# yang-z-03/scd-resnet

Hardware: AMD Instinct MI355X
Metric: 512x512 images/sec training, centerOffsetRes10, at 1/2/4/8 MI355X (higher is better)
Workload: dtype bf16; 1 GPU; centerOffsetRes10 train step (fwd+focal/L1 loss+bwd+Adam, DDP over RCCL), 512x512 synthetic SCD tiles; model=centerOffsetRes10, global_batch=32, step_issue=eager launches, per_gpu_batch=32, parallelism=dp1, image_size=512

## Files before the change

include/scdhip.h:

```cpp
#ifndef SCDHIP_H
#define SCDHIP_H
#include <stddef.h>
#include <stdint.h>

#ifdef __cplusplus
extern "C" {
#endif

#define SCD_DT_F32 0
#define SCD_DT_BF16 1
#define SCD_DT_F16 2

#define SCD_ERR_ARG 9001

#define SCD_MAX_TAPS 16
#define SCD_MAX_PHASES 4
#define SCD_STAT_REPLICAS 64

typedef struct scd_gemm_phase {
    int Qh, Qw, rho_h, rho_w, ntaps;
    int dh[SCD_MAX_TAPS], dw[SCD_MAX_TAPS], wt[SCD_MAX_TAPS];
} scd_gemm_phase;

int scd_conv_gemm(int dtype, const void* x, const void* w, void* y, const float* bias, double* stats,
                  int N, int Hi, int Wi, int Ci, int Ho, int Wo, int Co, int in_stride, int out_stride,
                  int wrow, int relu, int accumulate, int nphase, const scd_gemm_phase* phases,
                  void* stream);

int scd_conv_dgrad_s2(int dtype, const void* dy, const void* w3, void* dx, int N, int Hq, int Wq, int Cg, int Cin,
                      int accumulate, void* stream);
int scd_conv_gemm_bnbwd(int dtype, const void* x, const void* w, void* y, int N, int Hi, int Wi, int Ci, int Ho,
                        int Wo, int Co, int in_stride, int out_stride, int wrow, int nphase,
                        const scd_gemm_phase* phases, const void* bn_y, const float* mean, const float* invstd,
                        const float* relu_scale, const float* relu_shift, double* bn_stats, void* stream);
int scd_conv_gemm_res(int dtype, const void* x, const void* w, void* y, const float* bias, const void* res, int N,
                      int Hi, int Wi, int Ci, int Ho, int Wo, int Co, int in_stride, int out_stride, int wrow,
                      int relu, int nphase, const scd_gemm_phase* phases, void* stream);
int scd_conv_gemm_heads(int dtype, const void* x, const void* w, void* hid, const float* bias, int N, int H,
                        int W, int Ci, int nh, const int* od, const float* const* w1, const float* const* b1,
                        float* const* outs, void* stream);
int scd_conv_gemm_heads_keep(int dtype, const void* x, const void* w, void* hid, const float* bias, int N, int H,
                             int W, int Ci, int nh, const int* od, const float* const* w1, const float* const* b1,
                             float* const* outs, const unsigned char* keep, int keep_cols, void* stream);

size_t scd_conv_wgrad_workspace(int Cg, int T, int Ci, int nsplit);
int scd_conv_wgrad_nsplit(int dtype, long M, int Cg, int T, int Ci);
int scd_conv_wgrad_nsplit2(int dtype, long M, int Ho, int Wo, int Cg, int T, int Ci);
int scd_conv_wgrad(int dtype, const void* g, const void* x, float* ws, int nsplit,
                   int N, int Ho, int Wo, int Cg, int Hi, int Wi, int Ci, int in_stride,
                   int T, const int* dh, const int* dw, void* stream);
int scd_wgrad_reduce(const float* ws, int nsplit, int Cg, int T, int Ci, int r0, int r1, int cvalid,
                     long ld_n, long ld_c, long ld_t, float* dst, int accumulate, float alpha, void* stream);
int scd_wgrad_reduce_rows(const float* ws, int nsplit, int Cg, int T, int Ci, int nslices, const int* r0,
                          const int* r1, const long* ld_n, const long* ld_c, const long* ld_t, float* const* dst,
                          int cvalid, int accumulate, float alpha, void* stream);

int scd_pack_weight(int dtype, const float* w, void* out, int A, int B, int T, int mode, int ldp,
                    int row_off, void* stream);

int scd_pad_channels(int dtype, const void* src, long rows, int C, int Cp, void* dst, void* stream);

int scd_upsample2x_add(int dtype, const void* up, const void* low, void* out, int N, int h, int w, int C, void* stream);
int scd_upsample2x_add_bwd(int dtype, const void* dout, void* dlow, int N, int h, int w, int C, void* stream);

typedef struct scd_pack_desc {
    const float* w;
    void* out;
    long start;
    int A, B, T, mode, ldp, row_off, a_off, a_tot;
} scd_pack_desc;
int scd_pack_weights_batched(int dtype, const scd_pack_desc* descs, int n, long total, void* stream);

int scd_im2col_stem(int dtype, const float* x, void* cols, int N, int H, int W, int Ho, int Wo, int kh,
                    int kw, int stride, int pad, int Kpad, void* stream);

int scd_stem_conv_fwd(int dtype, const float* x, const void* wpk, void* y, double* stats, int N, int H, int W,
                      int Ho, int Wo, void* stream);
int scd_stem_conv_wgrad_nsplit(long M);
int scd_stem_conv_wgrad(int dtype, const void* dy, const void* ybn, const float* coef, const float* x, float* ws,
                        int nsplit, int N, int H, int W, int Ho, int Wo, void* stream);
int scd_stem_bwd_nsplit(void);
int scd_stem_bwd_fused(int dtype, const void* dout, const uint8_t* argmax, const void* y, const float* scale,
                       const float* shift, const float* mean, const float* invstd, const float* x, double* stats,
                       float* ws, int nsplit, float* tg, int N, int H, int W, int Ho, int Wo, void* stream);
int scd_stem_bwd_combine(int dtype, const float* tg, const void* wpk, const float* coef, float* dst, int accumulate,
                         float alpha, void* stream);

int scd_stats_collapse(double* stats, int nrep, int C, void* stream);
int scd_stats_collapse_to(double* stats, int nrep, int C, double* out, void* stream);
int scd_bn_finalize(double* stats, int nrep, int C, double count, const float* gamma,
                    const float* beta, float* running_mean, float* running_var, int64_t* num_batches,
                    float momentum, float eps, float* mean, float* invstd, float* scale, float* shift,
                    void* stream);
#define SCD_BN_FIN_MAX 4
typedef struct scd_bn_fin_args {
    double* stats;
    int nrep, C;
    double count;
    const float* gamma;
    const float* beta;
    float* running_mean;
    float* running_var;
    int64_t* num_batches;
    float momentum, eps;
    float* mean;
    float* invstd;
    float* scale;
    float* shift;
} scd_bn_fin_args;
int scd_bn_finalize_n(const scd_bn_fin_args* layers, int n, void* stream);
int scd_bn_apply(int dtype, const void* y, void* out, int C, long total, const float* scale,
                 const float* shift, const void* res, const float* rscale, const float* rshift,
                 int relu, void* stream);
int scd_bn_bwd_reduce(int dtype, const void* dout, const void* mask, const void* y, const float* relu_scale,
                      const float* relu_shift, const float* mean, const float* invstd, int C, long total,
                      double* stats, void* stream);
int scd_bn_bwd_finalize(double* stats, int nrep, int C, double count, const float* gamma,
// ... 189 lines not shown
```

scd-resnet_amd/csrc/conv_gemm.hip:

```cpp
#include <stdlib.h>

#include <algorithm>
#include <type_traits>

#include "gemm_common.h"
#include "scd_common.h"

#ifndef SCD_ABLATE
#define SCD_ABLATE 0
#endif

extern unsigned long long* scd_calib_stamp_buffer;

namespace {
SCD_KERNEL_NS_BEGIN

struct GemmParams {
    const char* x;
    const char* w;
    char* y;
    const float* bias;
    double* stats;
    int N, Hi, Wi, Ci, Ho, Wo, Co;
    int is, os, wrow, relu, accumulate, nphase, ntn;
// ... 819 lines not shown
        b_row[j] = b_ok[j] ? nn : 0;
    }
    const int cpt = p.Ci / BK;
    const int KT = ph.ntaps * cpt;
    const __amdgpu_buffer_rsrc_t xrs = buf_rsrc(p.x, p.xbytes);
    const __amdgpu_buffer_rsrc_t wrs = buf_rsrc(p.w, p.wbytes);

    struct StageArgs { int live, c0, dh, dw, wt; };
    auto stage_args = [&](int kt_req) {
        StageArgs a;
        a.live = kt_req < KT;
        const int kt = min(kt_req, KT - 1);
        const int chunk = kt / ph.ntaps, tap = kt - chunk * ph.ntaps;
        a.c0 = chunk * BK + cch * EPC;
        a.dh = ph.dh[tap]; a.dw = ph.dw[tap]; a.wt = ph.wt[tap];
        return a;
    };
    auto issue = [&](const StageArgs& g, int slot) {
        char* As = smem + slot * STAGE;
        char* Bs = As + BM * 128;
#pragma unroll
        for (int i = 0; i < 4; ++i) {
            const int ih = a_ih[i] + g.dh, iw = a_iw[i] + g.dw;
            const bool ok = g.live && a_ok[i] && (unsigned)ih < (unsigned)p.Hi && (unsigned)iw < (unsigned)p.Wi;
            dma16(xrs, As + (32 * wave + 8 * i) * 128, sel_off(ok, ((a_pix[i] + ih * p.Wi + iw) * p.Ci + g.c0) * 2));
        }
#pragma unroll
        for (int j = 0; j < 2; ++j)
            dma16(wrs, Bs + (16 * wave + 8 * j) * 128,
                  sel_off(g.live && b_ok[j], (b_row[j] * p.wrow + g.wt * p.Ci + g.c0) * 2));
    };

    const int wm = wave / WN, wn = wave - (wave / WN) * WN;
    const int l16 = lane & 15, lg = lane >> 4;
    const int l7 = l16 & 7;
    f32x4 acc[4][4];
#pragma unroll
    for (int a = 0; a < 4; ++a)
#pragma unroll
        for (int b = 0; b < 4; ++b) acc[a][b] = (f32x4){0.f, 0.f, 0.f, 0.f};

    issue(stage_args(0), 0);
    issue(stage_args(1), 1);
    int slot = 0;
    for (int kt = 0; kt < KT; ++kt) {
        const StageArgs nxt = stage_args(kt + 2);
        asm volatile("s_waitcnt vmcnt(6)" ::: "memory");
        __builtin_amdgcn_s_barrier();
        asm volatile("" ::: "memory");
        if constexpr (SCD_ABLATE == 2) asm volatile("s_waitcnt vmcnt(0)" ::: "memory");
        else issue(nxt, slot == 0 ? 2 : slot - 1);
        const char* As = smem + slot * STAGE;
        const char* Bs = As + BM * 128;
        h16x8 af[2][4], bfr[2][4];
#pragma unroll
        for (int s = 0; s < 2; ++s) {
            const int co = ((s * 4 + lg) ^ l7) << 4;
#pragma unroll
            for (int a = 0; a < 4; ++a) af[s][a] = *(const h16x8*)(As + (wm * 64 + a * 16 + l16) * 128 + co);
#pragma unroll
            for (int b = 0; b < 4; ++b) bfr[s][b] = *(const h16x8*)(Bs + (wn * 64 + b * 16 + l16) * 128 + co);
        }
        if constexpr (SCD_ABLATE == 1) {
#pragma unroll
            for (int s = 0; s < 2; ++s)
#pragma unroll
                for (int a = 0; a < 4; ++a) acc[a][0][0] += (float)af[s][a][0] + (float)bfr[s][a][0];
        } else {
            __builtin_amdgcn_s_setprio(1);
#pragma unroll
            for (int s = 0; s < 2; ++s)
#pragma unroll
                for (int a = 0; a < 4; ++a)
#pragma unroll
                    for (int b = 0; b < 4; ++b)
                        acc[a][b] = mfma_16x16x32_h16(bfr[s][b], af[s][a], acc[a][b]);
            __builtin_amdgcn_s_setprio(0);
        }
        slot = slot == 2 ? 0 : slot + 1;
    }
    asm volatile("s_waitcnt vmcnt(0)" ::: "memory");
    __syncthreads();
    gemm_epilogue<T, BM, BN, WN, HEADS, BNB, RES>(p, acc, smem, tid, bid, mt, nt, M, QQ, ph);
}

template <int BN, bool HEADS, bool BNB = false, bool RES = false>
__global__ __launch_bounds__(512, 1) void conv_gemm_pp_kernel(GemmParams p) {
    typedef h16 T;
    constexpr int BM = 256, BK = 64, EPC = 8;
    constexpr int NB = BN / 64;
    constexpr int WCOLS = BN / 4;
    constexpr int NB2 = (BN / 2 - 64) / 32;
    constexpr int STAGE = (BM + BN) * 128;
    constexpr int EROW = WCOLS * 2 + 16;
    constexpr int EPI = 8 * 128 * EROW;
    constexpr int EPX = EPI + 4 * BN * 4 + (HEADS ? 256 * 8 * 4 : 0);
    constexpr int SMEM = (2 * STAGE > EPX) ? 2 * STAGE : EPX;
    static_assert(BN == 256 || BN == 192, "BN");
    __shared__ __attribute__((aligned(16))) char smem[SMEM];

    const int tid = threadIdx.x;
    const int lane = tid & 63;
    const int wave = __builtin_amdgcn_readfirstlane(tid >> 6);
    const int grp = wave >> 2, wc = wave & 3;
    const int bid = xcd_tile_id();
    const GemmTile tile = gemm_tile(p, bid);
    const scd_gemm_phase& ph = p.ph[tile.phase];
    const int mt = tile.mt, nt = tile.nt, QQ = tile.QQ, M = tile.M;

    const int lrow = lane >> 3;
    const int cch = (lane & 7) ^ lrow;
    int a_base[4];
    unsigned a_mask[4];
#pragma unroll
    for (int i = 0; i < 4; ++i) {
        const int m = mt * BM + 128 * grp + 64 * (i >> 1) + 16 * wc + 8 * (i & 1) + lrow;
        const bool ok = m < M;
        const PixPos q = pix_of(ok ? m : 0, QQ, ph.Qw);
        const int ih0 = p.is * q.qh, iw0 = p.is * q.qw;
        a_base[i] = ((q.n * p.Hi + ih0) * p.Wi + iw0) * p.Ci * 2 + cch * EPC * 2;
        unsigned msk = 0;
        for (int t = 0; t < ph.ntaps; ++t) {
            const int ih = ih0 + ph.dh[t], iw = iw0 + ph.dw[t];
            if (ok && (unsigned)ih < (unsigned)p.Hi && (unsigned)iw < (unsigned)p.Wi) msk |= 1u << t;
        }
        a_mask[i] = msk;
    }
    int b_base[2 + NB2];
    bool b_ok[2 + NB2];
#pragma unroll
    for (int j = 0; j < 2 + NB2; ++j) {
        const int r = (BN / 2) * grp + (j < 2 ? 16 * wc + 8 * j : 64 + 8 * NB2 * wc + 8 * (j - 2)) + lrow;
        const int nn = nt * BN + r;
        b_ok[j] = nn < p.Co;
        b_base[j] = ((b_ok[j] ? nn : 0) * p.wrow + cch * EPC) * 2;
    }
    const int cpt = p.Ci / BK;
    const int KT = ph.ntaps * cpt;
    const __amdgpu_buffer_rsrc_t xrs = buf_rsrc(p.x, p.xbytes);
    const __amdgpu_buffer_rsrc_t wrs = buf_rsrc(p.w, p.wbytes);

    struct StageArgs { int live, tap, adelta, bdelta; };
    auto stage_args = [&](int kt_req) {
        StageArgs a;
        a.live = kt_req < KT;
        const int kt = min(kt_req, KT - 1);
        const int chunk = kt / ph.ntaps, tap = kt - chunk * ph.ntaps;
        a.tap = tap;
        a.adelta = ((ph.dh[tap] * p.Wi + ph.dw[tap]) * p.Ci + chunk * BK) * 2;
        a.bdelta = (ph.wt[tap] * p.Ci + chunk * BK) * 2;
        return a;
    };
    auto issue_a = [&](const StageArgs& g, char* buf, int h) {
#pragma unroll
        for (int j = 0; j < 2; ++j) {
            const int i = 2 * h + j;
            const bool ok = g.live && ((a_mask[i] >> g.tap) & 1u);
            dma16(xrs, buf + (128 * grp + 64 * h + 16 * wc + 8 * j) * 128, sel_off(ok, a_base[i] + g.adelta));
        }
    };
    auto issue_b = [&](const StageArgs& g, char* buf, int part) {
        char* Bs = buf + BM * 128;
#pragma unroll
        for (int j = (part ? 2 : 0); j < (part ? 2 + NB2 : 2); ++j) {
            const int r = (BN / 2) * grp + (j < 2 ? 16 * wc + 8 * j : 64 + 8 * NB2 * wc + 8 * (j - 2));
            dma16(wrs, Bs + r * 128, sel_off(g.live && b_ok[j], b_base[j] + g.bdelta));
// ... 1845 lines not shown
        if (bn == 256) hipLaunchKernelGGL((conv_gemm_pp_kernel<256, false, true>), dim3(tiles), dim3(512), 0, st, p);
        else hipLaunchKernelGGL((conv_gemm_pp_kernel<192, false, true>), dim3(tiles), dim3(512), 0, st, p);
    } else if (p.res) {
        if (bn == 256) hipLaunchKernelGGL((conv_gemm_pp_kernel<256, false, false, true>), dim3(tiles), dim3(512), 0, st, p);
        else hipLaunchKernelGGL((conv_gemm_pp_kernel<192, false, false, true>), dim3(tiles), dim3(512), 0, st, p);
    } else {
        if (bn == 256) hipLaunchKernelGGL((conv_gemm_pp_kernel<256, false>), dim3(tiles), dim3(512), 0, st, p);
        else hipLaunchKernelGGL((conv_gemm_pp_kernel<192, false>), dim3(tiles), dim3(512), 0, st, p);
    }
    SCD_RETURN_LAUNCH();
}

static int halo64_taps(const GemmParams& p, int nphase, const scd_gemm_phase* phases) {
    if (nphase != 1 || p.Ci != 64 || p.Co != 64 || p.is != 1 || p.os != 1 || p.head_on || p.wrow != 9 * 64) return -1;
    const scd_gemm_phase& ph = phases[0];
    if (ph.ntaps != 9 || ph.rho_h || ph.rho_w || ph.Qh != p.Ho || ph.Qw != p.Wo || p.Hi != p.Ho || p.Wi != p.Wo)
        return -1;
    if (p.Wo != 256 && p.Wo != 128 && p.Wo != 64) return -1;
    if (p.Wo < 256 && ph.Qh % (256 / p.Wo)) return -1;
    int fwd = 1, bwd = 1;
    for (int t = 0; t < 9; ++t) {
        const int r = t / 3, c = t % 3;
        if (ph.wt[t] != t) return -1;
        fwd &= ph.dh[t] == r - 1 && ph.dw[t] == c - 1;
        bwd &= ph.dh[t] == 1 - r && ph.dw[t] == 1 - c;
    }
    return fwd ? 0 : (bwd ? 1 : -1);
}

static int launch_l1p(int dtype, GemmParams& p, int nphase, const scd_gemm_phase* phases, long ,
                      hipStream_t st) {
    const int flip = halo64_taps(p, nphase, phases);
    const bool l1res = p.resmode && (p.bias || p.relu || p.res);
    if (dtype != SCD_DT_BF16 || flip < 0 || !halo64_mode() ||
        !(l1res ? (flip == 0 && !p.stats && !p.accumulate && !p.bnbwd) : (!p.bias && !p.relu && !p.res)))
        return -1;
    if (p.Wo == 256 && p.bnbwd) return SCD_ERR_ARG;
    const int tiles = fill_tiles(p, nphase, phases, 256, 1);
    if (!fill_ranges(dtype, p, l1res)) return SCD_ERR_ARG;
    const int tpi = p.Wo >= 256 ? p.Ho : p.Ho / (256 / p.Wo);
    int run = 1;
    while (run < 16 && tpi % (2 * run) == 0 && tiles / (2 * run) >= num_cus()) run *= 2;
    const int grid = tiles / run;
#define SCD_L1P_LAUNCH(WO)                                                                                              \
    do {                                                                                                                 \
        if (l1res) {                                                                                                     \
            hipLaunchKernelGGL((conv_gemm_l1p_kernel<WO, false, false, true>), dim3(grid), dim3(512), 0, st, p, run);    \
        } else if (WO != 256 && p.bnbwd) {                                                                                      \
            if (flip) hipLaunchKernelGGL((conv_gemm_l1p_kernel<WO, true, WO != 256>), dim3(grid), dim3(512), 0, st, p, run); \
            else hipLaunchKernelGGL((conv_gemm_l1p_kernel<WO, false, WO != 256>), dim3(grid), dim3(512), 0, st, p, run);    \
        } else {                                                                                                         \
            if (flip) hipLaunchKernelGGL((conv_gemm_l1p_kernel<WO, true, false>), dim3(grid), dim3(512), 0, st, p, run);  \
            else hipLaunchKernelGGL((conv_gemm_l1p_kernel<WO, false, false>), dim3(grid), dim3(512), 0, st, p, run);     \
        }                                                                                                                \
    } while (0)
    if (p.Wo == 256) SCD_L1P_LAUNCH(256);
    else if (p.Wo == 128) SCD_L1P_LAUNCH(128);
    else SCD_L1P_LAUNCH(64);
#undef SCD_L1P_LAUNCH
    SCD_RETURN_LAUNCH();
}

static int launch_ring(int dtype, GemmParams& p, int nphase, const scd_gemm_phase* phases, long Mtot,
                       hipStream_t st) {
    if (dtype != SCD_DT_BF16) return -1;
    bool ring;
    if (p.Co > 64) {
        const int rm = ring_mode();
        ring = rm >= 0 ? rm != 0 : cdiv(Mtot, 256) * cdiv(p.Co, 128) >= 256;
    } else {
        ring = nphase == 1 && phases[0].ntaps == 1 && p.Ci >= 128 && cdiv(Mtot, 256) >= 256;
    }
    if (!ring) return -1;
    const int tiles = fill_tiles(p, nphase, phases, 256, cdiv(p.Co, 128));
    if (tiles == 0) return 0;
    if (!fill_ranges(dtype, p, false)) return SCD_ERR_ARG;
    if (p.head_on) hipLaunchKernelGGL((conv_gemm_ring_kernel<true>), dim3(tiles), dim3(512), 0, st, p);
    else if (p.bnbwd) hipLaunchKernelGGL((conv_gemm_ring_kernel<false, true>), dim3(tiles), dim3(512), 0, st, p);
    else if (p.res) hipLaunchKernelGGL((conv_gemm_ring_kernel<false, false, true>), dim3(tiles), dim3(512), 0, st, p);
    else hipLaunchKernelGGL((conv_gemm_ring_kernel<false>), dim3(tiles), dim3(512), 0, st, p);
    SCD_RETURN_LAUNCH();
}

static int launch_tiled(int dtype, GemmParams& p, int nphase, const scd_gemm_phase* phases, long ,
                        hipStream_t st) {
    const bool narrow = p.Co <= 64;
    const int tiles = fill_tiles(p, nphase, phases, narrow ? 256 : 128, cdiv(p.Co, narrow ? 64 : 128));
    if (tiles == 0) return 0;
    if (!fill_ranges(dtype, p, false)) return SCD_ERR_ARG;
    return scd_dispatch_dtype(dtype, [&](auto tag) {
        using T = typename decltype(tag)::type;
        if (narrow) return launch_gemm<T, 256, 64>(p, tiles, st);
        int ks = 1;
        if (sizeof(T) == 2 && !p.head_on) {
            int kt = 0;
            for (int i = 0; i < nphase; ++i) kt = std::max(kt, phases[i].ntaps * (p.Ci / 64));
            if (kt >= 16 && 2 * (long)tiles <= 3L * num_cus()) ks = 2;
        }
        return launch_gemm<T, 128, 128>(p, tiles, st, ks);
    });
}

static int conv_gemm_launch(int dtype, GemmParams& p, int nphase, const scd_gemm_phase* phases, void* stream) {
    if (nphase < 1 || nphase > SCD_MAX_PHASES) return SCD_ERR_ARG;
    const int BK = dtype == SCD_DT_BF16 ? 64 : 32;
    const int EPC = dtype == SCD_DT_BF16 ? 8 : 4;
    if (p.Ci % BK != 0 || p.Co <= 0 || p.Co % EPC != 0 || p.N <= 0) return SCD_ERR_ARG;
    p.nphase = nphase;
    if (p.head_on && (p.Co <= 64 || p.Co != 128 * ((p.Co + 127) / 128))) return SCD_ERR_ARG;
    long Mtot = 0;
    for (int i = 0; i < nphase; ++i) {
        if (phases[i].ntaps < 0 || phases[i].ntaps > SCD_MAX_TAPS) return SCD_ERR_ARG;
        for (int t = 0; t < phases[i].ntaps; ++t)
            if (phases[i].wt[t] < 0 || (long)(phases[i].wt[t] + 1) * p.Ci > p.wrow) return SCD_ERR_ARG;
        Mtot += (long)p.N * phases[i].Qh * phases[i].Qw;
    }
    hipStream_t st = (hipStream_t)stream;
    int rc = launch_stream1x1(dtype, p, nphase, phases, Mtot, st);
    if (rc < 0 && stream1x1_mode() == 2) return SCD_ERR_ARG;
    if (rc < 0) rc = launch_heads384(dtype, p, nphase, phases, Mtot, st);
    if (rc < 0) rc = launch_pp(dtype, p, nphase, phases, Mtot, st);
    if (rc >= 0) return rc;
    if (p.bnbwd && dtype != SCD_DT_BF16) return SCD_ERR_ARG;
    rc = launch_l1p(dtype, p, nphase, phases, Mtot, st);
    if (rc < 0) rc = launch_ring(dtype, p, nphase, phases, Mtot, st);
    if (rc < 0) rc = launch_tiled(dtype, p, nphase, phases, Mtot, st);
    return rc;
}

static void fill_params(GemmParams& p, const void* x, const void* w, void* y, const float* bias, double* stats, int N,
                        int Hi, int Wi, int Ci, int Ho, int Wo, int Co, int in_stride, int out_stride, int wrow,
                        int relu, int accumulate) {
    p.x = (const char*)x; p.w = (const char*)w; p.y = (char*)y; p.bias = bias; p.stats = stats;
    p.N = N; p.Hi = Hi; p.Wi = Wi; p.Ci = Ci; p.Ho = Ho; p.Wo = Wo; p.Co = Co;
    p.is = in_stride; p.os = out_stride; p.wrow = wrow; p.relu = relu; p.accumulate = accumulate;
    p.ybytes = 0;
    p.head_on = 0;
    p.bnbwd = 0; p.bny = nullptr; p.bn_mean = p.bn_invstd = p.bn_rsc = p.bn_rsh = nullptr;
    p.hid_keep = nullptr; p.hid_cols = 1 << 30;
    p.shuf = 0;
    p.stamps = scd_calib_stamp_buffer;
    p.res = nullptr; p.resmode = 0;
    p.kserp = heads_serp_mode();
    for (int h = 0; h < 4; ++h) { p.head_od[h] = 0; p.head_w[h] = nullptr; p.head_b[h] = nullptr; p.head_out[h] = nullptr; }
}

extern "C" int scd_conv_gemm(int dtype, const void* x, const void* w, void* y, const float* bias, double* stats,
                             int N, int Hi, int Wi, int Ci, int Ho, int Wo, int Co, int in_stride, int out_stride,
                             int wrow, int relu, int accumulate, int nphase, const scd_gemm_phase* phases,
                             void* stream) {
    SCD_F16_FWD(scd_conv_gemm, x, w, y, bias, stats, N, Hi, Wi, Ci, Ho, Wo, Co, in_stride, out_stride, wrow, relu,
                accumulate, nphase, phases, stream);
    GemmParams p;
    fill_params(p, x, w, y, bias, stats, N, Hi, Wi, Ci, Ho, Wo, Co, in_stride, out_stride, wrow, relu, accumulate);
    return conv_gemm_launch(dtype, p, nphase, phases, stream);
}

extern "C" int scd_conv_gemm_res(int dtype, const void* x, const void* w, void* y, const float* bias, const void* res,
                                 int N, int Hi, int Wi, int Ci, int Ho, int Wo, int Co, int in_stride, int out_stride,
                                 int wrow, int relu, int nphase, const scd_gemm_phase* phases, void* stream) {
    SCD_F16_FWD(scd_conv_gemm_res, x, w, y, bias, res, N, Hi, Wi, Ci, Ho, Wo, Co, in_stride, out_stride, wrow, relu,
                nphase, phases, stream);
    if (res && res == y) return SCD_ERR_ARG;
    GemmParams p;
    fill_params(p, x, w, y, bias, nullptr, N, Hi, Wi, Ci, Ho, Wo, Co, in_stride, out_stride, wrow, relu, 0);
    p.res = (const char*)res; p.resmode = 1;
    return conv_gemm_launch(dtype, p, nphase, phases, stream);
}

extern "C" int scd_conv_gemm_bnbwd(int dtype, const void* x, const void* w, void* y, int N, int Hi, int Wi, int Ci,
                                   int Ho, int Wo, int Co, int in_stride, int out_stride, int wrow, int nphase,
                                   const scd_gemm_phase* phases, const void* bn_y, const float* mean,
                                   const float* invstd, const float* relu_scale, const float* relu_shift,
                                   double* bn_stats, void* stream) {
    SCD_F16_FWD(scd_conv_gemm_bnbwd, x, w, y, N, Hi, Wi, Ci, Ho, Wo, Co, in_stride, out_stride, wrow, nphase, phases,
                bn_y, mean, invstd, relu_scale, relu_shift, bn_stats, stream);
    if (!bn_y || !mean || !invstd || !relu_scale || !relu_shift || !bn_stats || Co % 4) return SCD_ERR_ARG;
    GemmParams p;
    fill_params(p, x, w, y, nullptr, bn_stats, N, Hi, Wi, Ci, Ho, Wo, Co, in_stride, out_stride, wrow, 0, 0);
    p.bnbwd = 1;
    p.bny = (const char*)bn_y; p.bn_mean = mean; p.bn_invstd = invstd; p.bn_rsc = relu_scale; p.bn_rsh = relu_shift;
    if (dtype == SCD_DT_BF16) {
        const int rc = conv_gemm_launch(dtype, p, nphase, phases, stream);
        if (rc != SCD_ERR_ARG) return rc;
    }
    fill_params(p, x, w, y, nullptr, nullptr, N, Hi, Wi, Ci, Ho, Wo, Co, in_stride, out_stride, wrow, 0, 0);
    const int rc = conv_gemm_launch(dtype, p, nphase, phases, stream);
    if (rc) return rc;
    return scd_bn_bwd_reduce(dtype, y, nullptr, bn_y, relu_scale, relu_shift, mean, invstd, Co, (long)N * Ho * Wo * Co,
                             bn_stats, stream);
}

extern "C" int scd_conv_dgrad_s2(int dtype, const void* dy, const void* w3, void* dx, int N, int Hq, int Wq, int Cg,
                                 int Cin, int accumulate, void* stream) {
    SCD_F16_FWD(scd_conv_dgrad_s2, dy, w3, dx, N, Hq, Wq, Cg, Cin, accumulate, stream);
    const int Co = 4 * Cin;
    if (!pp_tile_bn(dtype, Co, (long)N * Hq * Wq) || Cin % 8) return SCD_ERR_ARG;
    GemmParams p;
    fill_params(p, dy, w3, dx, nullptr, nullptr, N, Hq, Wq, Cg, Hq, Wq, Co, 1, 1, 4 * Cg, 0, accumulate);
    p.shuf = 1;
    scd_gemm_phase ph;
    ph.Qh = Hq; ph.Qw = Wq; ph.rho_h = 0; ph.rho_w = 0; ph.ntaps = 4;
    for (int t = 0; t < 4; ++t) { ph.dh[t] = t >> 1; ph.dw[t] = t & 1; ph.wt[t] = t; }
    return conv_gemm_launch(dtype, p, 1, &ph, stream);
}

extern "C" int scd_conv_gemm_heads(int dtype, const void* x, const void* w, void* hid, const float* bias, int N,
                                   int H, int W, int Ci, int nh, const int* od, const float* const* w1,
                                   const float* const* b1, float* const* outs, void* stream) {
    SCD_F16_FWD(scd_conv_gemm_heads, x, w, hid, bias, N, H, W, Ci, nh, od, w1, b1, outs, stream);
    return scd_conv_gemm_heads_keep(dtype, x, w, hid, bias, N, H, W, Ci, nh, od, w1, b1, outs, nullptr, 0, stream);
}

extern "C" int scd_conv_gemm_heads_keep(int dtype, const void* x, const void* w, void* hid, const float* bias, int N,
                                        int H, int W, int Ci, int nh, const int* od, const float* const* w1,
                                        const float* const* b1, float* const* outs, const unsigned char* keep,
                                        int keep_cols, void* stream) {
    SCD_F16_FWD(scd_conv_gemm_heads_keep, x, w, hid, bias, N, H, W, Ci, nh, od, w1, b1, outs, keep, keep_cols, stream);
    if (nh < 1 || nh > 4 || (keep && (keep_cols < 0 || keep_cols % 128))) return SCD_ERR_ARG;
    GemmParams p;
    fill_params(p, x, w, hid, bias, nullptr, N, H, W, Ci, H, W, nh * 128, 1, 1, 9 * Ci, 1, 0);
    if (keep) { p.hid_keep = keep; p.hid_cols = keep_cols; }
    p.head_on = 1;
    for (int h = 0; h < nh; ++h) {
        if (od[h] < 1 || od[h] > 4) return SCD_ERR_ARG;
        p.head_od[h] = od[h]; p.head_w[h] = w1[h]; p.head_b[h] = b1[h]; p.head_out[h] = outs[h];
    }
    scd_gemm_phase ph;
    ph.Qh = H; ph.Qw = W; ph.rho_h = 0; ph.rho_w = 0; ph.ntaps = 9;
    for (int t = 0; t < 9; ++t) { ph.dh[t] = t / 3 - 1; ph.dw[t] = t % 3 - 1; ph.wt[t] = t; }
    return conv_gemm_launch(dtype, p, 1, &ph, stream);
}

static void wgrad_tile(int Cg, int& tm, int& tn) {
    if (Cg <= 64) { tm = 64; tn = 256; }
    else { tm = 128; tn = 128; }
}

// ... 284 lines not shown
```

scd-resnet_amd/csrc/scd_common.h:

```cpp
#pragma once
#include <hip/hip_runtime.h>
#include <stdint.h>
#include <string.h>

#include "../../include/scdhip.h"

#define SCD_F16_ENTRY_POINTS(X) \
    X(scd_conv_gemm) \
    X(scd_conv_gemm_bnbwd) \
    X(scd_conv_gemm_res) \
    X(scd_conv_gemm_heads) \
    X(scd_conv_gemm_heads_keep) \
    X(scd_conv_wgrad_nsplit2) \
    X(scd_conv_wgrad_nsplit) \
    X(scd_conv_wgrad) \
    X(scd_bn_apply) \
    X(scd_bn_bwd_reduce) \
    X(scd_bn_bwd_apply) \
    X(scd_bn_bwd_reduce2) \
    X(scd_bn_bwd_apply2) \
    X(scd_pack_weights_batched) \
    X(scd_pack_weight) \
    X(scd_im2col_stem) \
    X(scd_stem_pool_fwd) \
    X(scd_stem_pool_bwd) \
    X(scd_stem_pool_bwd_bn) \
    X(scd_heads_fwd) \
    X(scd_heads_bwd) \
    X(scd_heads_bwd_packed) \
    X(scd_heads_bwd_packed_split) \
    X(scd_heads_sparse_bwd) \
    X(scd_heads_sparse_fixup) \
    X(scd_stem_conv_fwd) \
    X(scd_stem_conv_wgrad) \
    X(scd_stem_bwd_fused) \
    X(scd_conv_dgrad_s2) \
    X(scd_stem_bwd_combine) \
    X(scd_pad_channels) \
    X(scd_upsample2x_add) \
    X(scd_upsample2x_add_bwd)
#ifdef SCD_F16_BUILD
#define SCD_F16_RENAME(fn) extern "C" decltype(fn) fn __asm__(#fn "__f16");
SCD_F16_ENTRY_POINTS(SCD_F16_RENAME)
#define SCD_F16_FWD(fn, ...) ((void)0)
#else
#define SCD_F16_DECL(fn) extern "C" decltype(fn) fn##__f16;
SCD_F16_ENTRY_POINTS(SCD_F16_DECL)
#define SCD_F16_FWD(fn, ...) \
    do { if (dtype == SCD_DT_F16) return fn##__f16(SCD_DT_BF16, __VA_ARGS__); } while (0)
#endif

#ifdef SCD_F16_BUILD
#define SCD_KERNEL_NS_BEGIN inline namespace f16 {
#define SCD_KERNEL_NS_END }
#else
#define SCD_KERNEL_NS_BEGIN
#define SCD_KERNEL_NS_END
#endif

__device__ __forceinline__ float h16_word_half(unsigned w, int hi) {
#ifdef SCD_F16_BUILD
    return (float)__builtin_bit_cast(_Float16, (unsigned short)(hi ? w >> 16 : w & 0xffffu));
#else
    return __uint_as_float(hi ? (w & 0xffff0000u) : (w << 16));
#endif
}

typedef __attribute__((ext_vector_type(4))) float f32x4;
typedef __attribute__((ext_vector_type(8))) __bf16 bf16x8;
#ifdef SCD_F16_BUILD
typedef _Float16 h16;
#else
typedef __bf16 h16;
#endif
typedef __attribute__((ext_vector_type(8))) h16 h16x8;
typedef __attribute__((ext_vector_type(4))) h16 h16x4;
__device__ __forceinline__ f32x4 mfma_16x16x32_h16(h16x8 a, h16x8 b, f32x4 c) {
#ifdef SCD_F16_BUILD
    return __builtin_amdgcn_mfma_f32_16x16x32_f16(a, b, c, 0, 0, 0);
#else
    return __builtin_amdgcn_mfma_f32_16x16x32_bf16(a, b, c, 0, 0, 0);
#endif
}
typedef __attribute__((ext_vector_type(4))) short s16x4;
typedef __attribute__((address_space(3))) s16x4 lds_s16x4;

template <typename T> struct scd_type { using type = T; };
template <typename F>
static inline int scd_dispatch_dtype(int dtype, F&& f) {
    if (dtype == SCD_DT_BF16) return f(scd_type<h16>{});
#ifndef SCD_F16_BUILD
// ... 74 lines not shown
```

scd-resnet_amd/scdhip/lib.py:

```python
import ctypes
import os

import torch

HERE = os.path.dirname(os.path.abspath(__file__))
LIB_PATH = os.environ.get("SCDHIP_LIB", os.path.join(HERE, "libscdhip.so"))

DT_F32 = 0
DT_BF16 = 1
DT_F16 = 2
MAX_TAPS = 16
MAX_PHASES = 4
STAT_REPLICAS = 64

c_int, c_long, c_float, c_double, c_size_t, c_void_p = (ctypes.c_int, ctypes.c_long, ctypes.c_float,
                                                        ctypes.c_double, ctypes.c_size_t, ctypes.c_void_p)


class GemmPhase(ctypes.Structure):
    _fields_ = [("Qh", c_int), ("Qw", c_int), ("rho_h", c_int), ("rho_w", c_int), ("ntaps", c_int),
                ("dh", c_int * MAX_TAPS), ("dw", c_int * MAX_TAPS), ("wt", c_int * MAX_TAPS)]


class BnFinArgs(ctypes.Structure):
    _fields_ = [("stats", c_void_p), ("nrep", c_int), ("C", c_int), ("count", c_double), ("gamma", c_void_p),
                ("beta", c_void_p), ("running_mean", c_void_p), ("running_var", c_void_p), ("num_batches", c_void_p),
                ("momentum", c_float), ("eps", c_float), ("mean", c_void_p), ("invstd", c_void_p), ("scale", c_void_p),
                ("shift", c_void_p)]


class BnBwdFinArgs(ctypes.Structure):
    _fields_ = [("stats", c_void_p), ("nrep", c_int), ("C", c_int), ("count", c_double), ("gamma", c_void_p),
                ("mean", c_void_p), ("invstd", c_void_p), ("dgamma", c_void_p), ("dbeta", c_void_p),
                ("gscale", c_float), ("coef", c_void_p)]


class PackDesc(ctypes.Structure):
    _fields_ = [("w", c_void_p), ("out", c_void_p), ("start", c_long), ("A", c_int), ("B", c_int), ("T", c_int),
                ("mode", c_int), ("ldp", c_int), ("row_off", c_int), ("a_off", c_int), ("a_tot", c_int)]


P = c_void_p
I = c_int
L = c_long
F = c_float
D = c_double
PP = ctypes.POINTER(c_void_p)
IP = ctypes.POINTER(c_int)
LP = ctypes.POINTER(c_long)

SIGNATURES = {
    "scd_conv_gemm": (I, [I, P, P, P, P, P, I, I, I, I, I, I, I, I, I, I, I, I, I, ctypes.POINTER(GemmPhase), P]),
    "scd_conv_gemm_res": (I, [I, P, P, P, P, P, I, I, I, I, I, I, I, I, I, I, I, I, ctypes.POINTER(GemmPhase), P]),
    "scd_conv_gemm_heads": (I, [I, P, P, P, P, I, I, I, I, I, IP, PP, PP, PP, P]),
    "scd_conv_gemm_heads_keep": (I, [I, P, P, P, P, I, I, I, I, I, IP, PP, PP, PP, P, I, P]),
    "scd_conv_gemm_bnbwd": (I, [I, P, P, P, I, I, I, I, I, I, I, I, I, I, I, ctypes.POINTER(GemmPhase), P, P, P, P,
                                P, P, P]),
    "scd_conv_wgrad_workspace": (c_size_t, [I, I, I, I]),
    "scd_conv_wgrad_nsplit": (I, [I, L, I, I, I]),
    "scd_conv_wgrad_nsplit2": (I, [I, L, I, I, I, I, I]),
    "scd_conv_wgrad": (I, [I, P, P, P, I, I, I, I, I, I, I, I, I, I, IP, IP, P]),
    "scd_wgrad_reduce": (I, [P, I, I, I, I, I, I, I, L, L, L, P, I, F, P]),
    "scd_wgrad_reduce_rows": (I, [P, I, I, I, I, I, IP, IP, LP, LP, LP, PP, I, I, F, P]),
    "scd_pack_weight": (I, [I, P, P, I, I, I, I, I, I, P]),
    "scd_pack_weights_batched": (I, [I, P, I, L, P]),
    "scd_pad_channels": (I, [I, P, L, I, I, P, P]),
    "scd_upsample2x_add": (I, [I, P, P, P, I, I, I, I, P]),
    "scd_upsample2x_add_bwd": (I, [I, P, P, I, I, I, I, P]),
    "scd_im2col_stem": (I, [I, P, P, I, I, I, I, I, I, I, I, I, I, P]),
    "scd_stem_conv_fwd": (I, [I, P, P, P, P, I, I, I, I, I, P]),
    "scd_stem_conv_wgrad_nsplit": (I, [L]),
    "scd_stem_conv_wgrad": (I, [I, P, P, P, P, P, I, I, I, I, I, I, P]),
    "scd_stem_bwd_nsplit": (I, []),
    "scd_conv_dgrad_s2": (I, [I, P, P, P, I, I, I, I, I, I, P]),
    "scd_stem_bwd_fused": (I, [I, P, P, P, P, P, P, P, P, P, P, I, P, I, I, I, I, I, P]),
    "scd_stem_bwd_combine": (I, [I, P, P, P, P, I, F, P]),
    "scd_stem_pool_bwd_bn": (I, [I, P, P, P, P, P, P, P, P, P, I, I, I, I, I, I, P]),
    "scd_stats_collapse": (I, [P, I, I, P]),
    "scd_stats_collapse_to": (I, [P, I, I, P, P]),
    "scd_bn_finalize": (I, [P, I, I, D, P, P, P, P, P, F, F, P, P, P, P, P]),
    "scd_bn_apply": (I, [I, P, P, I, L, P, P, P, P, P, I, P]),
    "scd_bn_bwd_reduce": (I, [I, P, P, P, P, P, P, P, I, L, P, P]),
    "scd_bn_bwd_finalize": (I, [P, I, I, D, P, P, P, P, P, F, P, P]),
    "scd_bn_finalize_n": (I, [ctypes.POINTER(BnFinArgs), I, P]),
    "scd_bn_bwd_finalize_n": (I, [ctypes.POINTER(BnBwdFinArgs), I, P]),
    "scd_bn_bwd_apply": (I, [I, P, P, P, P, P, P, I, L, P, P, P]),
    "scd_bn_bwd_reduce2": (I, [I, P, P, P, P, P, P, P, P, I, L, P, P, P]),
    "scd_bn_bwd_apply2": (I, [I, P, P, P, P, P, P, I, L, P, P, P]),
    "scd_stem_pool_fwd": (I, [I, P, P, P, P, P, I, I, I, I, I, I, P]),
    "scd_stem_pool_bwd": (I, [I, P, P, P, P, P, P, I, I, I, I, I, I, P]),
    "scd_heads_fwd": (I, [I, P, I, I, I, I, IP, PP, PP, PP, P]),
    "scd_heads_bwd_accsize": (c_size_t, [I, I, IP]),
    "scd_heads_bwd": (I, [I, P, I, I, I, I, IP, PP, PP, P, P, P]),
    "scd_heads_bwd_packed": (I, [I, P, I, I, I, I, IP, PP, PP, F, P, P, P, P]),
    "scd_heads_bwd_weight_finalize": (I, [P, I, I, IP, PP, PP, PP, I, F, P]),
    "scd_heads_bwd_packed_split": (I, [I, P, I, I, I, I, IP, I, PP, PP, F, P, P, P, P]),
    "scd_heads_sparse_bwd": (I, [I, P, P, I, I, I, I, I, I, IP, I, PP, PP, F, P, I, P, P, P, P, P, P]),
    "scd_heads_sparse_fixup": (I, [I, P, P, I, I, I, I, P, I, P, P, P, P, P, P, P, P, P]),
    "scd_focal_fwd": (I, [P, P, L, P, P, P]),
    "scd_l1_gather_fwd": (I, [P, I, I, I, P, P, P, I, I, I, P, P, P]),
    "scd_centernet_loss_finalize": (I, [P, I, P, I, P, P, P, P]),
    "scd_scale_by_device": (I, [P, L, P, I, P, P]),
    "scd_heads_keep_map": (I, [P, I, I, I, P, I, P, P]),
    "scd_centernet_loss_fwd": (I, [P, P, L, P, I, P, I, I, I, P, P, P, I, I, I, I, P, P, P, P, P, P, P, P]),
    "scd_centernet_loss_bwd_scale": (I, [P, L, I, I, P, I, P, I, P, I, P, P, P]),
    "scd_corner_ae_fwd": (I, [P, P, I, I, P, P, P, I, F, F, P, I, P, P, P, P, P, P]),
    "scd_corner_ae_bwd": (I, [P, P, I, I, P, P, P, I, P, P, P, P]),
    "scd_corner_pairs": (I, [P, P, P, P, P, P, P, P, P, P, I, I, I, F, I, P, P, P]),
    "scd_decode_workspace": (c_size_t, [I, I]),
    "scd_decode_topk": (I, [P, I, I, I, I, P, I, P, I, P, P, P, P, P, P, P, P]),
    "scd_augment_workspace": (c_size_t, [I]),
    "scd_augment_tiles": (I, [P, P, I, I, I, P, P, P, F, ctypes.c_ulonglong, P, P]),
    "scd_augment_tiles_indexed": (I, [P, L, P, P, I, I, I, P, P, P, F, ctypes.c_ulonglong, P, P]),
    "scd_pack_locs": (I, [P, P, P, I, P, P, I, I, I, P, P, P]),
    "scd_rotate_tiles": (I, [P, P, I, I, I, P, P]),
    "scd_rotate_tiles_mapped": (I, [P, P, I, I, I, P, I, P]),
    "scd_slide_workspace": (c_size_t, [I]),
    "scd_slide_tiles": (I, [P, I, I, I, I, I, I, I, I, I, I, P, P, P]),
    "scd_slide_detections": (I, [P, I, I, I, I, I, I, F, P, P, P, P]),
    "scd_slide_samples_workspace": (c_size_t, [I, I]),
    "scd_slide_samples": (I, [P, I, I, I, I, I, I, F, I, I, I, I, I, D, D, I, P, P, P, P, P, P, P, P, P]),
    "scd_slide_rotate_workspace": (c_size_t, [I, I]),
    "scd_slide_rotate_clips": (I, [P, I, I, I, I, I, I, I, I, ctypes.POINTER(c_double), I, P, P, P]),
    "scd_ceval_count": (I, [P, P, P, P, P, P, P, I, I, I, I, I, I, F, P, P]),
    "scd_ceval_emit": (I, [P, P, P, P, P, P, P, I, I, I, I, I, I, F, P, PP, P]),
    "scd_ceval_summary_workspace": (c_size_t, [L]),
    "scd_ceval_summary": (I, [PP, ctypes.POINTER(c_long), L, P, I, P, P, P]),
    "scd_adam_step": (I, [P, P, P, P, L, F, F, F, F, F, F, F, P]),
    "scd_adam_step_dev": (I, [P, P, P, P, L, P, F, F, F, F, P, P]),
    "scd_sgd_step_dev": (I, [P, P, P, L, P, F, F, F, I, F, P, P]),
    "scd_render_center_targets": (I, [P, P, I, I, I, F, P, P, P, P, P]),
    "scd_render_corner_targets": (I, [P, P, I, I, I, F, P, P, P, P, P, P, P]),
    "scd_render_corner_targets_split": (I, [P, P, I, I, I, F, P, P, P, P, P, P, I, P]),
    "scd_corner_tag_inds": (I, [P, P, I, I, I, P, P, P, P]),
    "scd_cpool_fwd": (I, [I, I, P, P, P, I, I, I, I, P]),
# ... 83 lines not shown
```

Before: 6100 images/s.

## Add 4-slot ring-buffered 128x128 conv GEMM kernel with in-block split-K

Adds a new bf16 128x128 conv GEMM kernel that runs a 4-slot LDS ring of async buffer loads and can interleave two K halves into separate accumulators, merged before a shared epilogue. It is dispatched after the existing 256-row ring path for tile counts of at least 256 when the split-K heuristic picks 2, aiming to hide global load latency better than the tiled kernel. A selector entry point is also added so either kernel can be forced for benchmarking. In exchange it uses more shared memory and an extra LDS exchange step to combine the per-wave accumulator halves in the epilogue.

```diff
diff --git a/include/scdhip.h b/include/scdhip.h
--- a/include/scdhip.h
+++ b/include/scdhip.h
@@ -33,6 +33,11 @@
                         int Wo, int Co, int in_stride, int out_stride, int wrow, int nphase,
                         const scd_gemm_phase* phases, const void* bn_y, const float* mean, const float* invstd,
                         const float* relu_scale, const float* relu_shift, double* bn_stats, void* stream);
+int scd_conv_gemm_sel(int dtype, int kernel, const void* x, const void* w, void* y, const float* bias, double* stats,
+                      int N, int Hi, int Wi, int Ci, int Ho, int Wo, int Co, int in_stride, int out_stride, int wrow,
+                      int relu, int accumulate, int nphase, const scd_gemm_phase* phases, const void* bn_y,
+                      const float* mean, const float* invstd, const float* relu_scale, const float* relu_shift,
+                      void* stream);
 int scd_conv_gemm_res(int dtype, const void* x, const void* w, void* y, const float* bias, const void* res, int N,
                       int Hi, int Wi, int Ci, int Ho, int Wo, int Co, int in_stride, int out_stride, int wrow,
                       int relu, int nphase, const scd_gemm_phase* phases, void* stream);
diff --git a/scd-resnet_amd/csrc/conv_gemm.hip b/scd-resnet_amd/csrc/conv_gemm.hip
--- a/scd-resnet_amd/csrc/conv_gemm.hip
+++ b/scd-resnet_amd/csrc/conv_gemm.hip
@@ -925,6 +925,157 @@
     asm volatile("s_waitcnt vmcnt(0)" ::: "memory");
     __syncthreads();
     gemm_epilogue<T, BM, BN, WN, HEADS, BNB, RES>(p, acc, smem, tid, bid, mt, nt, M, QQ, ph);
+}
+
+template <int KS, bool BNB = false>
+__global__ __launch_bounds__(512, 1) void conv_gemm_ring128_kernel(GemmParams p) {
+    typedef h16 T;
+    static_assert(KS == 1 || KS == 2, "split K by 1 or 2");
+    constexpr int BM = 128, BN = 128, BK = 64, EPC = 8;
+    constexpr int STAGE = (BM + BN) * 128;
+    constexpr int NSLOT = 4;
+    __shared__ __attribute__((aligned(16))) char smem[NSLOT * STAGE];
+
+    const int tid = threadIdx.x;
+    const int lane = tid & 63;
+    const int wave = __builtin_amdgcn_readfirstlane(tid >> 6);
+    const int bid = xcd_tile_id();
+    const GemmTile tile = gemm_tile(p, bid);
+    const scd_gemm_phase& ph = p.ph[tile.phase];
+    const int mt = tile.mt, nt = tile.nt, QQ = tile.QQ, M = tile.M;
+
+    const int lrow = lane >> 3;
+    const int cch = (lane & 7) ^ (lrow & 7);
+    int a_pix[2], a_ih[2], a_iw[2];
+    bool a_ok[2];
+#pragma unroll
+    for (int i = 0; i < 2; ++i) {
+        const int m = mt * BM + 16 * wave + 8 * i + lrow;
+        a_ok[i] = m < M;
+        const PixPos q = pix_of(a_ok[i] ? m : 0, QQ, ph.Qw);
+        a_pix[i] = q.n * p.Hi * p.Wi;
+        a_ih[i] = p.is * q.qh;
+        a_iw[i] = p.is * q.qw;
+    }
+    int b_row[2];
+    bool b_ok[2];
+#pragma unroll
+    for (int j = 0; j < 2; ++j) {
+        const int nn = nt * BN + 16 * wave + 8 * j + lrow;
+        b_ok[j] = nn < p.Co;
+        b_row[j] = b_ok[j] ? nn : 0;
+    }
+    const int cpt = p.Ci / BK;
+    const int ntaps = max(ph.ntaps, 1);
+    const int KT = ph.ntaps * cpt;
+    const int KTg = (KT + KS - 1) / KS;
+    const int NST = KS * KTg;
+    const __amdgpu_buffer_rsrc_t xrs = buf_rsrc(p.x, p.xbytes);
+    const __amdgpu_buffer_rsrc_t wrs = buf_rsrc(p.w, p.wbytes);
+
+    struct StageArgs { int live, c0, dh, dw, wt; };
+    auto stage_args = [&](int s) {
+        StageArgs a;
+        const int kt_req = KS == 1 ? s : (s & 1) * KTg + (s >> 1);
+        a.live = s < NST && kt_req < KT;
+        const int kt = max(0, min(kt_req, KT - 1));
+        const int chunk = kt / ntaps, tap = kt - chunk * ntaps;
+        a.c0 = chunk * BK + cch * EPC;
+        a.dh = ph.dh[tap]; a.dw = ph.dw[tap]; a.wt = ph.wt[tap];
+        return a;
+    };
+    auto issue = [&](const StageArgs& g, int slot) {
+        char* As = smem + slot * STAGE;
+        char* Bs = As + BM * 128;
+#pragma unroll
+        for (int i = 0; i < 2; ++i) {
+            const int ih = a_ih[i] + g.dh, iw = a_iw[i] + g.dw;
+            const bool ok = g.live && a_ok[i] && (unsigned)ih < (unsigned)p.Hi && (unsigned)iw < (unsigned)p.Wi;
+            dma16(xrs, As + (16 * wave + 8 * i) * 128, sel_off(ok, ((a_pix[i] + ih * p.Wi + iw) * p.Ci + g.c0) * 2));
+        }
+#pragma unroll
+        for (int j = 0; j < 2; ++j)
+            dma16(wrs, Bs + (16 * wave + 8 * j) * 128,
+                  sel_off(g.live && b_ok[j], (b_row[j] * p.wrow + g.wt * p.Ci + g.c0) * 2));
+    };
+
+    const int wm = wave >> 2, wn = wave & 3;
+    const int l16 = lane & 15, lg = lane >> 4;
+    const int l7 = l16 & 7;
+    f32x4 acc[4][2], acc2[KS == 2 ? 4 : 1][2];
+#pragma unroll
+    for (int a = 0; a < 4; ++a)
+#pragma unroll
+        for (int b = 0; b < 2; ++b) {
+            acc[a][b] = (f32x4){0.f, 0.f, 0.f, 0.f};
+            if constexpr (KS == 2) acc2[a][b] = (f32x4){0.f, 0.f, 0.f, 0.f};
+        }
+
+    int slot = 0;
+    auto step = [&](int s, f32x4 (&c)[4][2]) {
+        const StageArgs nxt = stage_args(s + NSLOT - 1);
+        asm volatile("s_waitcnt vmcnt(%0)" ::"n"(4 * (NSLOT - 2)) : "memory");
+        __builtin_amdgcn_s_barrier();
+        asm volatile("" ::: "memory");
+        issue(nxt, slot == 0 ? NSLOT - 1 : slot - 1);
+        const char* As = smem + slot * STAGE;
+        const char* Bs = As + BM * 128;
+        h16x8 af[2][4], bfr[2][2];
+#pragma unroll
+        for (int k = 0; k < 2; ++k) {
+            const int co = ((k * 4 + lg) ^ l7) << 4;
+#pragma unroll
+            for (int a = 0; a < 4; ++a) af[k][a] = *(const h16x8*)(As + (wm * 64 + a * 16 + l16) * 128 + co);
+#pragma unroll
+            for (int b = 0; b < 2; ++b) bfr[k][b] = *(const h16x8*)(Bs + (wn * 32 + b * 16 + l16) * 128 + co);
+        }
+        __builtin_amdgcn_s_setprio(1);
+#pragma unroll
+        for (int k = 0; k < 2; ++k)
+#pragma unroll
+            for (int a = 0; a < 4; ++a)
+#pragma unroll
+                for (int b = 0; b < 2; ++b) c[a][b] = mfma_16x16x32_h16(bfr[k][b], af[k][a], c[a][b]);
+        __builtin_amdgcn_s_setprio(0);
+        slot = slot == NSLOT - 1 ? 0 : slot + 1;
+    };
+
+#pragma unroll
+    for (int s = 0; s < NSLOT - 1; ++s) issue(stage_args(s), s);
+    for (int s = 0; s < NST; s += KS) {
+        step(s, acc);
+        if constexpr (KS == 2) step(s + 1, acc2);
+    }
+    asm volatile("s_waitcnt vmcnt(0)" ::: "memory");
+    __syncthreads();
+    if constexpr (KS == 2) {
+#pragma unroll
+        for (int a = 0; a < 4; ++a)
+#pragma unroll
+            for (int b = 0; b < 2; ++b) acc[a][b] += acc2[a][b];
+    }
+    float* xs = (float*)smem + (wave >> 1) * 32 * 64 + lane;
+    if (wave & 1) {
+#pragma unroll
+        for (int a = 0; a < 4; ++a)
+#pragma unroll
+            for (int b = 0; b < 2; ++b)
+#pragma unroll
+                for (int r = 0; r < 4; ++r) xs[(a * 8 + b * 4 + r) * 64] = acc[a][b][r];
+    }
+    __syncthreads();
+    if (wave & 1) return;
+    f32x4 full[4][4];
+#pragma unroll
+    for (int a = 0; a < 4; ++a)
+#pragma unroll
+        for (int b = 0; b < 2; ++b) {
+            full[a][b] = acc[a][b];
+#pragma unroll
+            for (int r = 0; r < 4; ++r) full[a][2 + b][r] = xs[(a * 8 + b * 4 + r) * 64];
+        }
+    __syncthreads();
+    gemm_epilogue<T, BM, BN, 2, false, BNB, false>(p, full, smem, ((wave >> 1) << 6) | lane, bid, mt, nt, M, QQ, ph);
 }
 
 template <int BN, bool HEADS, bool BNB = false, bool RES = false>
@@ -2936,6 +3087,34 @@
     SCD_RETURN_LAUNCH();
 }
 
+static int tile128_ksplit(const GemmParams& p, int nphase, const scd_gemm_phase* phases, int tiles) {
+    if (p.head_on) return 1;
+    int kt = 0;
+    for (int i = 0; i < nphase; ++i) kt = std::max(kt, phases[i].ntaps * (p.Ci / 64));
+    return kt >= 16 && 2 * (long)tiles <= 3L * num_cus() ? 2 : 1;
+}
+
+static int launch_ring128(int dtype, GemmParams& p, int nphase, const scd_gemm_phase* phases, long ,
+                          hipStream_t st, bool force = false) {
+    if (dtype != SCD_DT_BF16 || p.Co <= 64 || p.head_on || p.res || p.shuf) return -1;
+    const int ntn = cdiv(p.Co, 128);
+    long tiles = 0;
+    for (int i = 0; i < nphase; ++i) tiles += (long)cdiv((long)p.N * phases[i].Qh * phases[i].Qw, 128) * ntn;
+    if (tiles == 0 || tiles >= (1L << 30)) return -1;
+    const int ks = tile128_ksplit(p, nphase, phases, (int)tiles);
+    if (!force && (tiles < 256 || ks != 2)) return -1;
+    fill_tiles(p, nphase, phases, 128, ntn);
+    if (!fill_ranges(dtype, p, false)) return SCD_ERR_ARG;
+    if (ks == 2) {
+        if (p.bnbwd) hipLaunchKernelGGL((conv_gemm_ring128_kernel<2, true>), dim3(tiles), dim3(512), 0, st, p);
+        else hipLaunchKernelGGL((conv_gemm_ring128_kernel<2>), dim3(tiles), dim3(512), 0, st, p);
+    } else {
+        if (p.bnbwd) hipLaunchKernelGGL((conv_gemm_ring128_kernel<1, true>), dim3(tiles), dim3(512), 0, st, p);
+        else hipLaunchKernelGGL((conv_gemm_ring128_kernel<1>), dim3(tiles), dim3(512), 0, st, p);
+    }
+    SCD_RETURN_LAUNCH();
+}
+
 static int launch_tiled(int dtype, GemmParams& p, int nphase, const scd_gemm_phase* phases, long ,
                         hipStream_t st) {
     const bool narrow = p.Co <= 64;
@@ -2945,17 +3124,12 @@
     return scd_dispatch_dtype(dtype, [&](auto tag) {
         using T = typename decltype(tag)::type;
         if (narrow) return launch_gemm<T, 256, 64>(p, tiles, st);
-        int ks = 1;
-        if (sizeof(T) == 2 && !p.head_on) {
-            int kt = 0;
-            for (int i = 0; i < nphase; ++i) kt = std::max(kt, phases[i].ntaps * (p.Ci / 64));
-            if (kt >= 16 && 2 * (long)tiles <= 3L * num_cus()) ks = 2;
-        }
-        return launch_gemm<T, 128, 128>(p, tiles, st, ks);
+        return launch_gemm<T, 128, 128>(p, tiles, st, sizeof(T) == 2 ? tile128_ksplit(p, nphase, phases, tiles) : 1);
     });
 }
 
-static int conv_gemm_launch(int dtype, GemmParams& p, int nphase, const scd_gemm_phase* phases, void* stream) {
+static int conv_gemm_launch(int dtype, GemmParams& p, int nphase, const scd_gemm_phase* phases, void* stream,
+                            int sel = -1) {
     if (nphase < 1 || nphase > SCD_MAX_PHASES) return SCD_ERR_ARG;
     const int BK = dtype == SCD_DT_BF16 ? 64 : 32;
     const int EPC = dtype == SCD_DT_BF16 ? 8 : 4;
@@ -2970,6 +3144,12 @@
         Mtot += (long)p.N * phases[i].Qh * phases[i].Qw;
     }
     hipStream_t st = (hipStream_t)stream;
+    if (sel >= 0) {
+        if (dtype != SCD_DT_BF16 || p.Co <= 64 || sel > 1) return SCD_ERR_ARG;
+        const int rs = sel == 1 ? launch_ring128(dtype, p, nphase, phases, Mtot, st, true)
+                                : launch_tiled(dtype, p, nphase, phases, Mtot, st);
+        return rs < 0 ? SCD_ERR_ARG : rs;
+    }
     int rc = launch_stream1x1(dtype, p, nphase, phases, Mtot, st);
     if (rc < 0 && stream1x1_mode() == 2) return SCD_ERR_ARG;
     if (rc < 0) rc = launch_heads384(dtype, p, nphase, phases, Mtot, st);
@@ -2978,6 +3158,7 @@
     if (p.bnbwd && dtype != SCD_DT_BF16) return SCD_ERR_ARG;
     rc = launch_l1p(dtype, p, nphase, phases, Mtot, st);
     if (rc < 0) rc = launch_ring(dtype, p, nphase, phases, Mtot, st);
+    if (rc < 0) rc = launch_ring128(dtype, p, nphase, phases, Mtot, st);
     if (rc < 0) rc = launch_tiled(dtype, p, nphase, phases, Mtot, st);
     return rc;
 }
@@ -3008,6 +3189,24 @@
     GemmParams p;
     fill_params(p, x, w, y, bias, stats, N, Hi, Wi, Ci, Ho, Wo, Co, in_stride, out_stride, wrow, relu, accumulate);
     return conv_gemm_launch(dtype, p, nphase, phases, stream);
+}
+
+extern "C" int scd_conv_gemm_sel(int dtype, int kernel, const void* x, const void* w, void* y, const float* bias,
+                                 double* stats, int N, int Hi, int Wi, int Ci, int Ho, int Wo, int Co, int in_stride,
+                                 int out_stride, int wrow, int relu, int accumulate, int nphase,
+                                 const scd_gemm_phase* phases, const void* bn_y, const float* mean,
+                                 const float* invstd, const float* relu_scale, const float* relu_shift, void* stream) {
+    SCD_F16_FWD(scd_conv_gemm_sel, kernel, x, w, y, bias, stats, N, Hi, Wi, Ci, Ho, Wo, Co, in_stride, out_stride, wrow,
+                relu, accumulate, nphase, phases, bn_y, mean, invstd, relu_scale, relu_shift, stream);
+    if (kernel < 0 || kernel > 1) return SCD_ERR_ARG;
+    GemmParams p;
+    fill_params(p, x, w, y, bias, stats, N, Hi, Wi, Ci, Ho, Wo, Co, in_stride, out_stride, wrow, relu, accumulate);
+    if (bn_y) {
+        if (!mean || !invstd || !relu_scale || !relu_shift || !stats || bias || relu || accumulate) return SCD_ERR_ARG;
+        p.bnbwd = 1;
+        p.bny = (const char*)bn_y; p.bn_mean = mean; p.bn_invstd = invstd; p.bn_rsc = relu_scale; p.bn_rsh = relu_shift;
+    }
+    return conv_gemm_launch(dtype, p, nphase, phases, stream, kernel);
 }
 
 extern "C" int scd_conv_gemm_res(int dtype, const void* x, const void* w, void* y, const float* bias, const void* res,
diff --git a/scd-resnet_amd/csrc/scd_common.h b/scd-resnet_amd/csrc/scd_common.h
--- a/scd-resnet_amd/csrc/scd_common.h
+++ b/scd-resnet_amd/csrc/scd_common.h
@@ -7,6 +7,7 @@
 
 #define SCD_F16_ENTRY_POINTS(X) \
     X(scd_conv_gemm) \
+    X(scd_conv_gemm_sel) \
     X(scd_conv_gemm_bnbwd) \
     X(scd_conv_gemm_res) \
     X(scd_conv_gemm_heads) \
diff --git a/scd-resnet_amd/scdhip/lib.py b/scd-resnet_amd/scdhip/lib.py
--- a/scd-resnet_amd/scdhip/lib.py
+++ b/scd-resnet_amd/scdhip/lib.py
@@ -51,6 +51,8 @@
 
 SIGNATURES = {
     "scd_conv_gemm": (I, [I, P, P, P, P, P, I, I, I, I, I, I, I, I, I, I, I, I, I, ctypes.POINTER(GemmPhase), P]),
+    "scd_conv_gemm_sel": (I, [I, I, P, P, P, P, P, I, I, I, I, I, I, I, I, I, I, I, I, I, ctypes.POINTER(GemmPhase), P, P,
+                              P, P, P, P]),
     "scd_conv_gemm_res": (I, [I, P, P, P, P, P, I, I, I, I, I, I, I, I, I, I, I, I, ctypes.POINTER(GemmPhase), P]),
     "scd_conv_gemm_heads": (I, [I, P, P, P, P, I, I, I, I, I, IP, PP, PP, PP, P]),
     "scd_conv_gemm_heads_keep": (I, [I, P, P, P, P, I, I, I, I, I, IP, PP, PP, PP, P, I, P]),
```

New measurement: 6170 images/s, median of 6. 1.01x the previous value.
